# xiongzhenhai-zh/emqx

Measured on AMD Instinct MI355X. Metric: published topics matched/sec (and match evals/sec) at 10M subs; % of HBM BW, higher is better.
Workload: dtype u32; 1 GPU; B: 10M mixed exact/'+'/'#' subscriptions, 1xMI355X, batched topics of depth 4-8; n_filters=10000000, batch_topics_per_gpu=1000000, mode=routes, parallelism=replicated table, topic stream split x1, walk_order=batch order

## Files before the change

### emqx_amd/csrc/engine.cpp

```cpp
#include <hip/hip_runtime.h>

#include <algorithm>
#include <atomic>
#include <chrono>
#include <cstdlib>
#include <cstring>
#include <memory>
#include <mutex>
#include <string>
#include <thread>
#include <vector>

#include "../../include/emqx_match.h"
#include "kernels.h"
#include "streams.h"
#include "tables.h"

using namespace emqx;

namespace {

#define HIP_TRY(expr)                    \
  do {                                   \
    hipError_t _e = (expr);              \
// ... 99 lines not shown
  uint32_t deep_slab_cap = 1u << 20;
  uint64_t* h_rb = nullptr;
  bool deep_ready = false;
  bool ordered = false;
  hipEvent_t evo = nullptr;
  uint64_t ord_cap_n = 0, ord_cap_bytes = 0, ord_temp_bytes = 0;
  uint64_t* ord_keys = nullptr;
  uint64_t* ord_keys_out = nullptr;
  uint32_t* ord_idx = nullptr;
  uint32_t* ord_perm = nullptr;
  uint32_t* ord_lens = nullptr;
  uint32_t* ord_corig = nullptr;
  uint64_t* ord_noffs = nullptr;
  uint64_t* ord_partials = nullptr;
  uint8_t* ord_bytes = nullptr;
  uint8_t* ord_temp = nullptr;

  ~Workspace() {
    (void)hipSetDevice(device);
    dfree(counts); dfree(deferred); dfree(deep_rank); dfree(slab); dfree(tile_fill);
    dfree(tile_defer); dfree(spill); dfree(diag); dfree(ctrl); dfree(tile_sum); dfree(tile_stats);
    dfree(group_sum); dfree(group_stats);
    dfree(deep_wids); dfree(deep_stack); dfree(deep_slab);
    dfree(ord_keys); dfree(ord_keys_out); dfree(ord_idx); dfree(ord_perm); dfree(ord_lens); dfree(ord_corig);
    dfree(ord_noffs); dfree(ord_partials); dfree(ord_bytes); dfree(ord_temp);
    if (h_rb) (void)hipHostFree(h_rb);
    if (ev0) (void)hipEventDestroy(ev0);
    if (ev1) (void)hipEventDestroy(ev1);
    if (evk) (void)hipEventDestroy(evk);
    if (evo) (void)hipEventDestroy(evo);
    if (done) (void)hipEventDestroy(done);
    if (stream) (void)hipStreamDestroy(stream);
  }
};

uint64_t round_pow2(uint64_t x) {
  uint64_t p = 1;
  while (p < x) p <<= 1;
  return p;
}

}

struct emqx_engine {
  int device = 0;
  std::mutex writer;
  FilterStore store;
  uint64_t epoch = 0;
  double last_build_ms = 0;
  std::mutex snap_mu;
  std::shared_ptr<Snapshot> snap;
  std::mutex ws_mu;
  std::vector<std::unique_ptr<Workspace>> all_ws;
  std::vector<Workspace*> free_ws;
  std::atomic<uint64_t> last_evals{0}, last_deferred{0}, last_max_stack{0};
  std::atomic<double> last_match_ms{0};
  std::atomic<double> last_kernel_ms{0};
  std::atomic<int> forced_variant{-1};
  std::atomic<bool> diag_on{false};
  std::atomic<uint32_t> diag_stop{0};
  uint4* timeline = nullptr;
  uint64_t timeline_cap = 0;
  std::atomic<uint32_t> slab_hint{256};
  LiveState ls;
  std::vector<uint32_t> dirty;
  bool incremental = true;
  int64_t delta_max = -1;
  uint64_t last_commit_kind = 0;
  uint64_t last_relocations = 0, last_in_place = 0, last_patches = 0, last_new_slots = 0;
  double last_host_ms = 0;
  uint64_t last_extents = 0, last_vocab_slots = 0;
  double last_upload_ms = 0;
  std::mutex hb_mu;
  std::vector<emqx_host_batch*> hb_free;
  int commit_threads = std::max(1u, std::min(8u, std::thread::hardware_concurrency()));
  std::atomic<int> order{-1};
  std::atomic<int> order_level_bits{0};
  std::atomic<int> order_sort_bits{64};
  std::atomic<int> order_deal{1};
  std::atomic<uint64_t> last_ordered{0};
  std::atomic<uint64_t> order_bpt{48};
  std::atomic<double> last_order_ms{0};
  std::atomic<bool> small_batch{true};
};

namespace {

constexpr int EMQX_NEED_FULL = 1;

void publish(emqx_engine* e, std::shared_ptr<Snapshot> s) {
  std::lock_guard<std::mutex> g(e->snap_mu);
  e->snap = std::move(s);
}

int full_commit(emqx_engine* e) {
  auto vs = std::make_unique<VocabState>();
  std::vector<uint64_t> loc;
  std::vector<uint32_t> slot_ids;
  BuildOpts o;
  o.vocab = vs.get();
  o.fid_loc = &loc;
  o.slot_ids = &slot_ids;
  o.threads = e->commit_threads;
  HostTables ht;
  std::string err;
  if (!build_tables(e->store, o, ht, &err)) {
    set_last_error(err.c_str());
    return EMQX_ENOMEM;
  }
  const uint64_t n_slots = ht.edges.size();
  const uint64_t spare = std::min<uint64_t>(std::max<uint64_t>(1u << 20, n_slots / 2), MAX_SLOTS - n_slots);
  auto dt = std::make_shared<DeviceTables>();
  dt->device = e->device;
  dt->cap_slots = n_slots + spare;
  dt->n_vocab = ht.vocab.size();
  dt->cap_arena = ht.arena.size() + std::max<uint64_t>(1u << 20, ht.arena.size() / 4) + 16;
  HIP_TRY(dalloc(dt->edges, dt->cap_slots));
  HIP_TRY(dalloc(dt->fids, 2 * dt->cap_slots));
  HIP_TRY(dalloc(dt->vocab, dt->n_vocab));
  HIP_TRY(dalloc(dt->arena, dt->cap_arena));
  HIP_TRY(hipMemcpy(dt->edges, ht.edges.data(), n_slots * sizeof(EdgeSlot), hipMemcpyHostToDevice));
  HIP_TRY(hipMemcpy(dt->fids, ht.fids.data(), ht.fids.size() * sizeof(uint32_t), hipMemcpyHostToDevice));
  HIP_TRY(hipMemcpy(dt->vocab, ht.vocab.data(), ht.vocab.size() * sizeof(VocabSlot), hipMemcpyHostToDevice));
  HIP_TRY(hipMemcpy(dt->arena, ht.arena.data(), ht.arena.size(), hipMemcpyHostToDevice));
  HIP_TRY(hipStreamSynchronize(nullptr));

  auto s = std::make_shared<Snapshot>();
  s->dt = dt;
  s->tv.edges = dt->edges;
  s->tv.fids = dt->fids;
  s->tv.vocab = dt->vocab;
  s->tv.arena = dt->arena;
  s->tv.vocab_mask = ht.vocab_mask;
  s->tv.root_base = ht.root_base;
  s->tv.root_meta = ht.root_meta;
  s->tv.root_hash_fid = ht.root_hash_fid;
  s->tv.plus_mask = ht.plus_mask;
  s->n_nodes = ht.n_nodes;
  s->n_slots = n_slots;
  s->n_words = ht.n_words;
  s->max_depth = ht.max_depth;
  s->bytes = dt->bytes();
  uint32_t max_id = 0;
  for (uint32_t x : e->store.ext) max_id = std::max(max_id, x);
  s->narrow = slab_narrow_ok(max_id);

  LiveState& d = e->ls;
  d.device = e->device;
  d.dt = dt;
  d.vocab = std::move(vs);
  if (!d.lt) d.lt = std::make_unique<LiveTrie>();
  d.lt->adopt(ht, loc, slot_ids, spare, d.vocab.get());
  d.valid = true;
  d.inserted = 0;
  d.base_live = e->store.n_live;
  e->dirty.clear();
  publish(e, std::move(s));
  e->last_commit_kind = 0;
  return EMQX_OK;
}

int live_commit(emqx_engine* e) {
  LiveState& d = e->ls;
  LiveTrie& lt = *d.lt;
  const FilterStore& fs = e->store;
  std::vector<uint32_t> ids(e->dirty);
// ... 125 lines not shown
    HIP_TRY(dalloc(w->ctrl, CTRL_WORDS));
    HIP_TRY(dalloc(w->diag, DIAG_WORDS));
    HIP_TRY(hipMemset(w->diag, 0, DIAG_WORDS * sizeof(uint64_t)));
  }
  if (!w->deep_ready) {
    HIP_TRY(dalloc(w->deep_wids, uint64_t(DEEP_WAVES) * DEEP_MAX_LEVELS));
    HIP_TRY(dalloc(w->deep_stack, uint64_t(DEEP_WAVES) * w->deep_stack_cap));
    HIP_TRY(dalloc(w->deep_slab, w->deep_slab_cap));
    w->deep_ready = true;
  }
  if (n > w->cap_n) {
    const uint64_t cap = round_pow2(std::max<uint64_t>(n, 1024));
    HIP_TRY(dalloc(w->counts, cap));
    HIP_TRY(dalloc(w->deferred, cap));
    HIP_TRY(dalloc(w->deep_rank, cap));
    w->cap_n = cap;
  }
  const uint64_t ntiles = (n + TILE_TOPICS - 1) / TILE_TOPICS;
  if (ntiles > w->cap_tiles || w->cap_tiles == 0) {
    const uint64_t cap = round_pow2(std::max<uint64_t>(ntiles, 64));
    HIP_TRY(dalloc(w->tile_fill, cap));
    HIP_TRY(dalloc(w->tile_defer, cap));
    HIP_TRY(dalloc(w->tile_sum, cap));
    HIP_TRY(dalloc(w->tile_stats, cap));
    HIP_TRY(dalloc(w->group_sum, cap / GROUP_TILES + 1));
    HIP_TRY(dalloc(w->group_stats, cap / GROUP_TILES + 1));
    HIP_TRY(dalloc(w->spill, cap * w->spill_cap));
    w->cap_tiles = cap;
  }
  const uint64_t need_slab = std::max<uint64_t>(ntiles, 1) * w->slab_per_tile * entry_bytes;
  if (need_slab > w->cap_slab) {
    const uint64_t cap = need_slab;
    HIP_TRY(dalloc(w->slab, cap));
    w->cap_slab = cap;
  }
  return EMQX_OK;
}

constexpr uint64_t ORDER_MIN_N = 65536;

bool use_order(const emqx_engine* e, const Snapshot& snap, uint64_t n) {
  if (n > 0xFFFFFFFFull) return false;
  const int o = e->order.load();
  if (o >= 0) return o > 0 && n > 0;
  return snap.max_depth > 12 && n >= ORDER_MIN_N;
}

int ensure_order(emqx_engine* e, Workspace* w, uint64_t n, uint32_t sort_bits) {
  if (n > w->ord_cap_n) {
    const uint64_t cap = round_pow2(std::max<uint64_t>(n, 1024));
    HIP_TRY(dalloc(w->ord_keys, cap));
    HIP_TRY(dalloc(w->ord_keys_out, cap));
    HIP_TRY(dalloc(w->ord_idx, cap));
    HIP_TRY(dalloc(w->ord_perm, cap));
    HIP_TRY(dalloc(w->ord_lens, cap));
    HIP_TRY(dalloc(w->ord_corig, cap));
    HIP_TRY(dalloc(w->ord_noffs, cap + 1));
    HIP_TRY(dalloc(w->ord_partials, scan_partials(cap)));
    w->ord_cap_n = cap;
  }
  const uint64_t tb = order_sort_temp_bytes(n, sort_bits);
  if (!w->ord_temp || tb > w->ord_temp_bytes) {
    HIP_TRY(dalloc(w->ord_temp, tb));
    w->ord_temp_bytes = tb;
  }
  const uint64_t want = e->order_bpt.load() * n + 4096;
  if (!w->ord_bytes || w->ord_cap_bytes < want) {
    const uint64_t cap = std::max<uint64_t>(w->ord_cap_bytes, want);
    HIP_TRY(dalloc(w->ord_bytes, cap + 16));
    w->ord_cap_bytes = cap;
  }
  return EMQX_OK;
}

FastVariant pick_variant(const emqx_engine* e, const Snapshot& snap) {
  static const int env_forced = [] {
    const char* v = getenv("EMQX_FAST_VARIANT");
    return v ? atoi(v) : -1;
  }();
  const int fv = e->forced_variant.load();
  const int forced = fv >= 0 ? fv : env_forced;
  if (forced >= 0 && forced < FAST_NVARIANTS) return static_cast<FastVariant>(forced);
  return snap.max_depth > 12 ? FAST_K1_S512W : FAST_K1_S384B1;
}

MatchArgs match_args(emqx_engine* e, const Snapshot& snap, Workspace* w, uint32_t mode, const uint8_t* d_tbytes,
                     const uint64_t* d_toffs, uint64_t n, uint64_t* d_out_off, uint32_t* d_out_ids, uint64_t cap,
                     uint64_t* summary) {
  MatchArgs a{};
  a.tv = snap.tv;
  a.tbytes = d_tbytes;
  a.toffs = d_toffs;
  a.n = n;
  a.mode = mode;
  a.slab_cap = w->slab_per_tile;
  a.counts = w->counts;
  a.slab = w->slab;
  a.narrow = snap.narrow ? 1u : 0u;
  a.tile_fill = w->tile_fill;
  a.tile_defer = w->tile_defer;
  a.spill = w->spill;
  a.diag = e->diag_on.load() ? w->diag : nullptr;
  a.diag_stop = a.diag ? e->diag_stop.load() : 0u;
  a.timeline = a.diag && e->timeline && (n + TILE_TOPICS - 1) / TILE_TOPICS <= e->timeline_cap ? e->timeline : nullptr;
  a.spill_cap = w->spill_cap;
  a.ctrl = w->ctrl;
  a.deferred = w->deferred;
  a.deep_wids = w->deep_wids;
  a.deep_stack = w->deep_stack;
  a.deep_stack_cap = w->deep_stack_cap;
  a.deep_waves = DEEP_WAVES;
  a.deep_slab = w->deep_slab;
  a.deep_slab_cap = w->deep_slab_cap;
  a.tile_sum = w->tile_sum;
  a.tile_stats = w->tile_stats;
  a.group_sum = w->group_sum;
  a.group_stats = w->group_stats;
  a.ngroups = static_cast<uint32_t>((n + TILE_TOPICS * GROUP_TILES - 1) / (TILE_TOPICS * GROUP_TILES));
  a.deep_rank = w->deep_rank;
  a.out_off = d_out_off;
  a.out_ids = d_out_ids;
  a.out_cap = d_out_ids ? cap : 0;
  a.summary = summary;
  return a;
}

uint64_t slab_entry_bytes(const Snapshot& snap) {
  return snap.narrow ? sizeof(SlabNarrow::T) : sizeof(SlabWide::T);
}

int enqueue_match(emqx_engine* e, const Snapshot& snap, Workspace* w, uint32_t mode, const uint8_t* d_tbytes,
                  const uint64_t* d_toffs, uint64_t n, uint64_t* d_out_off, uint32_t* d_out_ids, uint64_t cap,
                  uint64_t* summary, hipStream_t s) {
  int rc = ensure_ws(w, n, slab_entry_bytes(snap));
  if (rc != EMQX_OK) return rc;
  MatchArgs a = match_args(e, snap, w, mode, d_tbytes, d_toffs, n, d_out_off, d_out_ids, cap, summary);
  const bool ordered = use_order(e, snap, n);
  const uint32_t sort_bits = static_cast<uint32_t>(std::min(64, std::max(1, e->order_sort_bits.load())));
  if (ordered) {
    rc = ensure_order(e, w, n, sort_bits);
    if (rc != EMQX_OK) return rc;
  }

  HIP_TRY(hipStreamWaitEvent(s, w->done, 0));
  w->last_stream = s;
  HIP_TRY(hipMemsetAsync(w->ctrl, 0, CTRL_WORDS * sizeof(uint32_t), s));
  w->ordered = ordered;
  if (ordered) {
    HIP_TRY(hipEventRecord(w->evo, s));
    OrderArgs o{};
    o.tbytes = d_tbytes;
    o.toffs = d_toffs;
    o.n = n;
    const int lb = e->order_level_bits.load();
    o.level_bits = static_cast<uint32_t>(lb > 0 ? std::min(lb, 32) : (snap.max_depth > 12 ? 4 : 8));
    o.sort_bits = sort_bits;
    o.keys = w->ord_keys;
    o.keys_out = w->ord_keys_out;
    o.idx = w->ord_idx;
    o.perm = w->ord_perm;
    o.lens = w->ord_lens;
    o.noffs = w->ord_noffs;
    o.partials = w->ord_partials;
    o.obytes = w->ord_bytes;
    o.cap_bytes = w->ord_cap_bytes;
    o.temp = w->ord_temp;
    o.temp_bytes = w->ord_temp_bytes;
    o.ctrl = w->ctrl;
    HIP_TRY(launch_order(o, s));
    a.tbytes = w->ord_bytes;
    a.toffs = w->ord_noffs;
    a.perm = w->ord_perm;
    a.deal = e->order_deal.load() ? 1u : 0u;
    a.corig = w->ord_corig;
    a.partials = w->ord_partials;
  }
  HIP_TRY(hipEventRecord(w->ev0, s));
  HIP_TRY(launch_match_fast(a, pick_variant(e, snap), s));
  HIP_TRY(hipEventRecord(w->evk, s));
  HIP_TRY(launch_match_deep(a, s));
  HIP_TRY(launch_assemble(a, s));
  HIP_TRY(hipEventRecord(w->ev1, s));
  HIP_TRY(hipEventRecord(w->done, s));
  return EMQX_OK;
}

int run_match(emqx_engine* e, const Snapshot& snap, Workspace* w, uint32_t mode, const uint8_t* d_tbytes,
              const uint64_t* d_toffs, uint64_t n, uint64_t* d_out_off, uint32_t* d_out_ids, uint64_t cap,
              uint64_t* n_out, hipStream_t s) {
  uint64_t* sum_dev = nullptr;
  HIP_TRY(hipHostGetDevicePointer(reinterpret_cast<void**>(&sum_dev), w->h_rb, 0));
  for (int attempt = 0; attempt < 8; ++attempt) {
    int rc = enqueue_match(e, snap, w, mode, d_tbytes, d_toffs, n, d_out_off, d_out_ids, cap, sum_dev, s);
    if (rc != EMQX_OK) return rc;
    HIP_TRY(hipStreamSynchronize(s));
    const uint64_t* sm = w->h_rb;
    const uint64_t flags = sm[SUM_FLAGS];
    const uint32_t err = static_cast<uint32_t>(sm[SUM_ERROR]);
    if (flags & SUM_F_ERROR) {
      set_last_error("topic longer than 65535 bytes on the deep path");
      return EMQX_EINVAL;
    }
    if (flags & SUM_F_RETRY) {
      if (sm[SUM_NEED_SLAB] > w->slab_per_tile) {
        const uint64_t need = sm[SUM_NEED_SLAB];
// ... 607 lines not shown
  }
  auto s = current(e);
  if (s) {
    out->n_nodes = s->n_nodes;
    out->n_slots = s->n_slots;
    out->n_words = s->n_words;
    out->table_bytes = s->bytes;
    out->max_depth = s->max_depth;
  }
  out->last_ordered = e->last_ordered.load();
  out->last_order_ms = e->last_order_ms.load();
  out->last_evals = e->last_evals.load();
  out->last_deferred = e->last_deferred.load();
  out->last_max_stack = e->last_max_stack.load();
  out->last_match_ms = e->last_match_ms.load();
  out->last_kernel_ms = e->last_kernel_ms.load();
  out->size = want;
  std::memcpy(dst, out, want);
  return EMQX_OK;
}

const char* emqx_strerror(int code) {
  switch (code) {
    case EMQX_OK: return "ok";
    case EMQX_EINVAL: return "invalid argument";
    case EMQX_ENOMEM: return "out of memory";
    case EMQX_EDEVICE: return g_last_error.empty() ? "device error" : g_last_error.c_str();
    case EMQX_EOVERFLOW: return "output capacity too small";
    case EMQX_ENOTFOUND: return "not found";
    case EMQX_ETOODEEP: return "topic frontier too deep";
    case EMQX_EBUSY: return "busy: every batch buffer is in use";
    default: return "unknown error";
  }
}

int emqx_set_tuning(emqx_engine* e, const char* key, int64_t value) {
  if (!e || !key) return EMQX_EINVAL;
  if (std::strcmp(key, "fast_variant") == 0) {
    if (value < -1 || value >= FAST_NVARIANTS) return EMQX_EINVAL;
    e->forced_variant.store(static_cast<int>(value));
    return EMQX_OK;
  }
  if (std::strcmp(key, "diag") == 0) {
    e->diag_on.store(value != 0);
    return EMQX_OK;
  }
  if (std::strcmp(key, "diag_stop") == 0) {
    e->diag_stop.store(static_cast<uint32_t>(value));
    return EMQX_OK;
  }
  if (std::strcmp(key, "timeline") == 0) {
    if (value < 0) return EMQX_EINVAL;
    HIP_TRY(hipSetDevice(e->device));
    HIP_TRY(hipDeviceSynchronize());
    dfree(e->timeline);
    e->timeline_cap = 0;
    if (value) {
      HIP_TRY(dalloc(e->timeline, static_cast<uint64_t>(value)));
      HIP_TRY(hipMemset(e->timeline, 0, static_cast<uint64_t>(value) * sizeof(uint4)));
      e->timeline_cap = static_cast<uint64_t>(value);
    }
    return EMQX_OK;
  }
  if (std::strcmp(key, "small_batch") == 0) {
    e->small_batch.store(value != 0);
    return EMQX_OK;
  }
  if (std::strcmp(key, "incremental") == 0) {
    std::lock_guard<std::mutex> g(e->writer);
    e->incremental = value != 0;
    return EMQX_OK;
  }
  if (std::strcmp(key, "commit_threads") == 0) {
    if (value < 1 || value > 256) return EMQX_EINVAL;
    std::lock_guard<std::mutex> g(e->writer);
    e->commit_threads = static_cast<int>(value);
    return EMQX_OK;
  }
  if (std::strcmp(key, "order") == 0) {
    if (value < -1 || value > 1) return EMQX_EINVAL;
    e->order.store(static_cast<int>(value));
    return EMQX_OK;
  }
  if (std::strcmp(key, "order_level_bits") == 0) {
    if (value < 0 || value > 32) return EMQX_EINVAL;
    e->order_level_bits.store(static_cast<int>(value));
    return EMQX_OK;
  }
  if (std::strcmp(key, "order_sort_bits") == 0) {
    if (value < 1 || value > 64) return EMQX_EINVAL;
    e->order_sort_bits.store(static_cast<int>(value));
    return EMQX_OK;
  }
  if (std::strcmp(key, "order_deal") == 0) {
    e->order_deal.store(value != 0);
    return EMQX_OK;
  }
  if (std::strcmp(key, "delta_max") == 0) {
    std::lock_guard<std::mutex> g(e->writer);
    e->delta_max = value;
    return EMQX_OK;
  }
  return EMQX_ENOTFOUND;
}

uint64_t emqx_permute_scratch_bytes(uint64_t n) { return permute_scratch_bytes(n); }

uint64_t emqx_owner_sort_scratch_bytes(uint64_t n, uint32_t world) { return owner_sort_scratch_bytes(n, world); }

int emqx_owner_sort_device(const uint32_t* d_owner, uint64_t n, uint32_t world, uint32_t* d_perm, void* d_scratch,
                           void* stream) {
  if (world == 0 || (n && (!d_owner || !d_perm || !d_scratch)) || n > 0xFFFFFFFFull) return EMQX_EINVAL;
  HIP_TRY(launch_owner_sort(d_owner, n, world, d_perm, d_scratch, static_cast<hipStream_t>(stream)));
  return EMQX_OK;
}

int emqx_batch_permute_device(const uint8_t* d_bytes, const uint64_t* d_offsets, uint64_t n, const uint32_t* d_perm,
                              uint8_t* d_out_bytes, uint64_t* d_out_offsets, void* d_scratch, void* stream) {
  if (!d_out_offsets || !d_scratch || (n && (!d_bytes || !d_offsets || !d_perm || !d_out_bytes))) return EMQX_EINVAL;
  HIP_TRY(launch_batch_permute(d_bytes, d_offsets, n, d_perm, d_out_bytes, d_out_offsets, d_scratch,
                               static_cast<hipStream_t>(stream)));
  return EMQX_OK;
}

int emqx_csr_unpermute_device(const uint32_t* d_counts, const uint32_t* d_ids, uint64_t n, const uint32_t* d_perm,
                              uint64_t* d_out_offsets, uint32_t* d_out_ids, void* d_scratch, void* stream) {
  if (!d_out_offsets || !d_scratch || (n && (!d_counts || !d_perm))) return EMQX_EINVAL;
  HIP_TRY(launch_csr_unpermute(d_counts, d_ids, n, d_perm, d_out_offsets, d_out_ids, d_scratch,
                               static_cast<hipStream_t>(stream)));
  return EMQX_OK;
}

int emqx_shard_owner_device(const uint8_t* d_bytes, const uint64_t* d_offsets, uint64_t n, uint32_t world,
                            uint32_t levels, uint32_t* d_owner, void* stream) {
  if ((n && (!d_bytes || !d_offsets || !d_owner)) || world == 0 || levels == 0) return EMQX_EINVAL;
  HIP_TRY(launch_shard_owner(d_bytes, d_offsets, n, world, levels, d_owner, static_cast<hipStream_t>(stream)));
  return EMQX_OK;
}

int emqx_shard_route_device(const uint8_t* d_bytes, const uint64_t* d_offsets, uint64_t n, uint32_t world,
                            const emqx_shard_split* d_splits, uint32_t n_splits, uint32_t* d_req2, void* stream) {
  if ((n && (!d_bytes || !d_offsets || !d_req2)) || world == 0 || (n_splits && !d_splits)) return EMQX_EINVAL;
  HIP_TRY(launch_shard_route(d_bytes, d_offsets, n, world, reinterpret_cast<const ShardSplitE*>(d_splits), n_splits,
                             d_req2, static_cast<hipStream_t>(stream)));
  return EMQX_OK;
}

int emqx_commit_stats(emqx_engine* e, uint64_t* out, uint32_t n) {
  if (!e || (n && !out)) return EMQX_EINVAL;
  std::lock_guard<std::mutex> g(e->writer);
  const LiveTrie* lt = e->ls.lt.get();
  uint64_t host_us = static_cast<uint64_t>(e->last_host_ms * 1e3);
  const uint64_t v[12] = {e->last_commit_kind, e->last_relocations, e->last_in_place, e->last_patches,
                          e->last_new_slots, lt ? lt->used : 0, lt ? lt->cap : 0, lt ? lt->garbage : 0, host_us,
                          e->last_extents, e->last_vocab_slots, static_cast<uint64_t>(e->last_upload_ms * 1e3)};
  for (uint32_t i = 0; i < n && i < 12; ++i) out[i] = v[i];
  return EMQX_OK;
}

int emqx_diag_read(emqx_engine* e, uint64_t* out, uint32_t n, int reset) {
  if (!e || !out) return EMQX_EINVAL;
  HIP_TRY(hipSetDevice(e->device));
  std::vector<uint64_t> acc(DIAG_WORDS, 0), tmp(DIAG_WORDS);
  std::lock_guard<std::mutex> g(e->ws_mu);
  for (auto& w : e->all_ws) {
    if (!w->diag) continue;
// ... 22 lines not shown
```

### emqx_amd/csrc/kernels.h

```cpp
#pragma once

#include <hip/hip_runtime.h>
#include <stdint.h>

#include "layout.h"

namespace emqx {

enum Ctrl : uint32_t {
  CTRL_DEFERRED = 0,
  CTRL_NEED_SLAB = 1,
  CTRL_ERROR = 2,
  CTRL_DEEP_FILL = 3,
  CTRL_DEEP_EVALS = 4,
  CTRL_WORDS = 8
};
constexpr uint32_t GROUP_TILES = 256;
constexpr uint32_t CTRL_ERR_TOO_LONG = 1u;
constexpr uint32_t CTRL_ERR_TOO_DEEP = 2u;
constexpr uint32_t CTRL_ERR_DEEP_SLAB = 4u;
constexpr uint32_t CTRL_ERR_ORDER_CAP = 8u;

constexpr int TILE_TOPICS = 64;

enum Diag : uint32_t {
  DIAG_STEPS = 0,
  DIAG_ITEMS = 1,
  DIAG_LIT_PROBES = 2,
  DIAG_LIT_HITS = 3,
  DIAG_LIT_EXTRA = 4,
  DIAG_PLUS_PROBES = 5,
  DIAG_PLUS_HITS = 6,
  DIAG_EMITS = 7,
  DIAG_SPILLS = 8,
  DIAG_TICKS_A = 9,
  DIAG_TICKS_B = 10,
  DIAG_WAVES = 11,
  DIAG_LEVEL0 = 12,
  DIAG_SMALL = 20,
  DIAG_WIDE = 21,
  DIAG_NCOUNT = 22,
  DIAG_WORDS = 32
};
constexpr uint32_t DEEP_MAX_LEVELS = 65536;

enum Summary : uint32_t {
  SUM_FLAGS = 0,
  SUM_TOTAL = 1,
  SUM_EVALS = 2,
  SUM_MAXSTACK = 3,
  SUM_DEFERRED = 4,
  SUM_NEED_SLAB = 5,
  SUM_DEEP_FILL = 6,
  SUM_ERROR = 7,
  SUM_WORDS = 8
};
constexpr uint64_t SUM_F_RETRY = 1;
constexpr uint64_t SUM_F_OVERFLOW = 2;
constexpr uint64_t SUM_F_ERROR = 4;

struct MatchArgs {
  TableView tv;
  const uint8_t* tbytes;
  const uint64_t* toffs;
  uint64_t n;
  uint32_t mode;
  uint32_t slab_cap;
  uint32_t* counts;
  void* slab;
  uint32_t narrow;
  uint32_t* tile_fill;
  uint64_t* tile_defer;
  uint32_t* ctrl;
  uint32_t* deferred;
  uint64_t* diag;
  uint4* timeline;
  uint32_t diag_stop;
  uint2* spill;
  uint32_t spill_cap;
  uint32_t* deep_wids;
  uint4* deep_stack;
  uint32_t deep_stack_cap;
  uint32_t deep_waves;
  uint64_t* deep_slab;
  uint32_t deep_slab_cap;
  uint64_t* tile_sum;
  uint2* tile_stats;
  uint64_t* group_sum;
  uint2* group_stats;
  uint32_t ngroups;
  uint32_t* deep_rank;
  uint64_t* out_off;
  uint32_t* out_ids;
  uint64_t out_cap;
  uint64_t* summary;
  const uint32_t* perm;
  uint32_t deal;
  uint32_t* corig;
  uint64_t* partials;
};

constexpr uint32_t SMALL_WAVES = 16;
constexpr uint64_t SMALL_MAX_N = uint64_t(SMALL_WAVES) * TILE_TOPICS;
constexpr uint32_t SMALL_FO_MAX_ENTRIES = 16384;

struct SmallFanout {
  const uint4* recs;
  uint32_t n_recs;
  const uint32_t* plain;
  const uint4* groups;
  const uint32_t* members;
  uint32_t strategy;
  uint32_t seed;
  const uint32_t* h_keys;
  uint32_t* d_keys;
  uint4* erec;
  uint32_t* etop;
  const unsigned long long* ps_count;
  uint64_t* h_off;
  uint32_t* h_subs;
  uint32_t* h_fil;
  uint64_t cap;
  uint64_t* h_sum;
};

struct SmallArgs {
  MatchArgs m;
  const uint8_t* h_tbytes;
  const uint64_t* h_toffs;
  uint64_t nbytes;
  uint32_t tt;
  uint32_t slab_tiles;
  uint32_t has_fanout;
  uint64_t* h_out_off;
  uint32_t* h_out_ids;
  uint64_t h_cap;
  uint64_t* clk;
  SmallFanout f;
};
enum : uint32_t {
  SMALL_CLK_COPY = 0, SMALL_CLK_WALK, SMALL_CLK_DEEP, SMALL_CLK_SCAN, SMALL_CLK_SCATTER, SMALL_CLK_OUT,
  SMALL_CLK_FO_PASS1, SMALL_CLK_FO_PASS2, SMALL_CLK_LAUNCHES, SMALL_CLK_WORDS = 10
};
hipError_t launch_small_batch(const SmallArgs& a, hipStream_t s);
}
struct emqx_engine;
namespace emqx {
constexpr int SMALL_NOT_TAKEN = 1;
int engine_small_batch(emqx_engine* e, uint32_t mode, const uint8_t* h_tbytes, const uint64_t* h_toffs, uint64_t n,
                       uint64_t nbytes, uint8_t* d_tbytes, uint64_t* d_toffs, uint64_t* d_out_off, uint32_t* d_out_ids,
                       uint64_t cap, uint64_t* h_summary, const SmallFanout& f, hipStream_t s);

constexpr uint32_t DEEP_WAVES = 512;
constexpr uint32_t DEEP_CHUNK = 256;
constexpr uint64_t DEEP_PAD = ~0ull;

enum FastVariant {
  FAST_K1_S1K = 0,
  FAST_K2_S1K = 1,
  FAST_K2_S2K = 2,
  FAST_K2_S768 = 3,
  FAST_K4_S2K = 4,
  FAST_K1_S256 = 5,
  FAST_K2_S512 = 6,
  FAST_K1_S384 = 7,
  FAST_K2_S512W = 8,
  FAST_K1_S768W = 9,
  FAST_K1_S512W = 10,
  FAST_K1_S384R = 11,
  FAST_K1_S384P = 12,
  FAST_K1_S384N = 13,
  FAST_K1_S384W7 = 14,
  FAST_K1_S384B2 = 15,
  FAST_K1_S384B1 = 16,
  FAST_K1_S512WB1 = 17,
  FAST_NVARIANTS = 18
};
// ... 49 lines not shown
```

### emqx_amd/csrc/layout.h

```cpp
#pragma once

#include <stdint.h>

#if defined(__HIPCC__)
#define EMQX_HD __host__ __device__ __forceinline__
#else
#define EMQX_HD inline
#endif

namespace emqx {

constexpr uint32_t WID_NONE = 0xFFFFFFFFu;
constexpr uint32_t WID_PLUS = 0xFFFFFFFEu;
constexpr uint32_t WID_HASH = 0xFFFFFFFDu;
constexpr uint32_t FID_NONE = 0xFFFFFFFFu;

constexpr uint32_t META_CAPLOG2_MASK = 0x1Fu;
constexpr uint32_t META_HAS_PLUS = 1u << 5;
constexpr uint32_t META_HAS_EDGES = 1u << 6;
constexpr uint32_t META_HAS_HASH = 1u << 7;
constexpr uint32_t META_HAS_TERM = 1u << 8;
constexpr uint32_t META_TERM_WILD = 1u << 9;
constexpr uint32_t META_PH = 1u << 10;
constexpr uint32_t META_LITF_EXACT = 1u << 11;
constexpr uint32_t META_LITF_NONE = 1u << 12;
constexpr uint32_t META_BUCKET_OVF = 1u << 13;
constexpr uint32_t META_XFID = 1u << 14;
constexpr uint32_t META_XFID_TERM = 1u << 15;
constexpr uint32_t META_F8_SHIFT = 24;
constexpr uint32_t META_SEED_SHIFT = 16;
constexpr uint32_t PH_MAX_CAPLOG = 15;

struct alignas(16) EdgeSlot {
  uint32_t wid;
  uint32_t child_base;
  uint32_t meta;
  uint32_t litf;
};
static_assert(sizeof(EdgeSlot) == 16, "EdgeSlot must be 16 bytes");
constexpr uint64_t MAX_SLOTS = (1ull << 31) - 1;

constexpr uint32_t SLAB_NARROW_ID_BITS = 26;
constexpr uint32_t SLAB_NARROW_IDS = (1u << SLAB_NARROW_ID_BITS) - 1u;
EMQX_HD bool slab_narrow_ok(uint32_t max_id) { return max_id < SLAB_NARROW_IDS; }
struct SlabWide {
  typedef uint64_t T;
  static constexpr T PAD = ~0ull;
  static EMQX_HD T make(uint32_t owner, uint32_t id) { return (static_cast<uint64_t>(owner) << 32) | id; }
  static EMQX_HD uint32_t owner(T e) { return static_cast<uint32_t>(e >> 32) & 63u; }
  static EMQX_HD uint32_t id(T e) { return static_cast<uint32_t>(e); }
};
struct SlabNarrow {
  typedef uint32_t T;
  static constexpr T PAD = ~0u;
  static EMQX_HD T make(uint32_t owner, uint32_t id) { return (owner << SLAB_NARROW_ID_BITS) | id; }
  static EMQX_HD uint32_t owner(T e) { return e >> SLAB_NARROW_ID_BITS; }
  static EMQX_HD uint32_t id(T e) { return e & ((1u << SLAB_NARROW_ID_BITS) - 1u); }
};

struct alignas(16) SlotPatch {
  uint32_t slot;
  uint32_t fid_h, fid_t;
  uint32_t pad;
  EdgeSlot s;
};
static_assert(sizeof(SlotPatch) == 32, "SlotPatch must be 32 bytes");

struct alignas(16) VocabSlot {
  uint32_t hash;
  uint32_t len;
  uint32_t wid;
  uint32_t off;
  uint32_t inl[4];
};
static_assert(sizeof(VocabSlot) == 32, "VocabSlot must be 32 bytes");

struct TableView {
  const EdgeSlot* edges;
  const uint32_t* fids;
  const VocabSlot* vocab;
  const uint8_t* arena;
  uint32_t vocab_mask;
  uint32_t root_base;
  uint32_t root_meta;
  uint32_t root_hash_fid;
  uint32_t plus_mask;
};

constexpr uint32_t PLUS_LINE = 4;
constexpr uint32_t PLUS_COPY_MAX_CAPLOG = 14;
EMQX_HD bool plus_copies(uint32_t plus_mask, bool has_plus, uint32_t caplog) {
  return plus_mask != 0 && has_plus && caplog > 2 && caplog <= PLUS_COPY_MAX_CAPLOG;
}
EMQX_HD bool plus_position(uint32_t i, bool copies) { return copies ? (i & (PLUS_LINE - 1u)) == 0 : i == 0; }
EMQX_HD uint32_t plus_copy(uint32_t i1, bool copies) { return copies ? (i1 & ~(PLUS_LINE - 1u)) : 0u; }

EMQX_HD uint32_t mix32(uint32_t x) {
  x ^= x >> 16;
  x *= 0x85ebca6bu;
  x ^= x >> 13;
  x *= 0xc2b2ae35u;
  x ^= x >> 16;
  return x;
}

EMQX_HD uint32_t whash_init(uint32_t len) { return len * 0x9E3779B1u + 0x7F4A7C15u; }
EMQX_HD uint32_t whash_step(uint32_t h, uint32_t d) {
  h = (h ^ d) * 0x85EBCA77u;
  return (h << 13) | (h >> 19);
}
EMQX_HD uint32_t word_hash16(uint32_t len, uint32_t w0, uint32_t w1, uint32_t w2, uint32_t w3) {
  return mix32(whash_step(whash_step(whash_step(whash_step(whash_init(len), w0), w1), w2), w3));
}
EMQX_HD uint32_t word_hash_bytes(const uint8_t* p, uint32_t n) {
  uint32_t h = whash_init(n);
  const uint32_t nd = n > 16 ? (n + 3) / 4 : 4;
  for (uint32_t i = 0; i < nd; ++i) {
    uint32_t d = 0;
    for (uint32_t b = 0; b < 4; ++b)
      if (4 * i + b < n) d |= static_cast<uint32_t>(p[4 * i + b]) << (8 * b);
    h = whash_step(h, d);
  }
  return mix32(h);
}

EMQX_HD uint32_t vocab_slot0(uint32_t hash) { return hash; }

EMQX_HD uint32_t node_hash(uint32_t wid, uint32_t seed) { return mix32(wid ^ (seed * 0x9E3779B1u + 0x7F4A7C15u)); }

EMQX_HD uint32_t ph_slot(uint32_t h, uint32_t mask, bool copies) {
  const uint32_t s = h & mask;
  return (!copies || (s & (PLUS_LINE - 1u))) ? s : s + 1u + (h >> 31);
}
EMQX_HD uint32_t lit_slot(uint32_t wid, uint32_t seed, uint32_t mask, bool copies) {
  return ph_slot(node_hash(wid, seed), mask, copies);
}


EMQX_HD uint32_t bucket1(uint32_t wid, uint32_t seed, uint32_t nbmask) { return node_hash(wid, seed) & nbmask; }
EMQX_HD uint32_t bucket2(uint32_t wid, uint32_t seed, uint32_t nbmask) {
  const uint32_t a = bucket1(wid, seed, nbmask), b = mix32(wid ^ (0xDAA66D2Bu + seed * 0x7F4A7C15u)) & nbmask;
// ... 201 lines not shown
```

### emqx_amd/csrc/match_kernels.hip

```cpp
#include <hip/hip_runtime.h>

#include <algorithm>

#include "fanout.h"
#include "kernels.h"

namespace emqx {

namespace {

constexpr uint32_t MODE_ROUTES = 0, MODE_TRIE = 1;

__device__ __forceinline__ uint32_t lane_id() {
  return __builtin_amdgcn_mbcnt_hi(~0u, __builtin_amdgcn_mbcnt_lo(~0u, 0u));
}

__device__ __forceinline__ void wave_sync() {
  __builtin_amdgcn_fence(__ATOMIC_SEQ_CST, "wavefront");
  __builtin_amdgcn_wave_barrier();
}

__device__ __forceinline__ uint64_t lanemask_lt(uint32_t lane) { return (1ull << lane) - 1ull; }

template <int BITS>
// ... 1198 lines not shown
#pragma unroll
  for (int k = 0; k < SCAN_ITEMS; ++k) {
    const uint64_t i = base + k;
    v[k] = i < n ? counts[i] : 0u;
    s += v[k];
  }
  uint64_t tot;
  uint64_t run = partials[blockIdx.x] + block_excl_scan(s, &tot);
#pragma unroll
  for (int k = 0; k < SCAN_ITEMS; ++k) {
    const uint64_t i = base + k;
    if (i < n) offsets[i] = run;
    run += v[k];
  }
}

__global__ __launch_bounds__(SCAN_THREADS) void scan_single_kernel(const uint32_t* counts, uint64_t n,
                                                                   uint64_t* offsets) {
  const uint64_t base = static_cast<uint64_t>(threadIdx.x) * SCAN_ITEMS;
  uint32_t v[SCAN_ITEMS];
  uint64_t s = 0;
#pragma unroll
  for (int k = 0; k < SCAN_ITEMS; ++k) {
    const uint64_t i = base + k;
    v[k] = i < n ? counts[i] : 0u;
    s += v[k];
  }
  uint64_t tot;
  uint64_t run = block_excl_scan(s, &tot);
#pragma unroll
  for (int k = 0; k < SCAN_ITEMS; ++k) {
    const uint64_t i = base + k;
    if (i < n) offsets[i] = run;
    run += v[k];
  }
  if (threadIdx.x == 0) offsets[n] = tot;
}

__device__ __forceinline__ uint64_t wave_sum64(uint64_t v) {
#pragma unroll
  for (uint32_t d = 32; d >= 1; d >>= 1)
    v += (static_cast<uint64_t>(__shfl_xor(static_cast<uint32_t>(v >> 32), d, 64)) << 32) |
         __shfl_xor(static_cast<uint32_t>(v), d, 64);
  return v;
}

__global__ __launch_bounds__(GROUP_TILES) void group_reduce_kernel(MatchArgs a, uint64_t ntiles) {
  __shared__ uint64_t ws[GROUP_TILES / 64], we[GROUP_TILES / 64];
  __shared__ uint32_t wm[GROUP_TILES / 64];
  const uint32_t lane = threadIdx.x & 63, w = threadIdx.x >> 6;
  const uint64_t i = static_cast<uint64_t>(blockIdx.x) * GROUP_TILES + threadIdx.x;
  uint64_t v = 0, ev = 0;
  uint32_t mx = 0;
  if (i < ntiles) {
    v = a.tile_sum[i];
    const uint2 st = a.tile_stats[i];
    ev = st.x;
    mx = st.y;
  }
  v = wave_sum64(v);
  ev = wave_sum64(ev);
  for (uint32_t d = 32; d >= 1; d >>= 1) mx = max(mx, static_cast<uint32_t>(__shfl_xor(mx, d, 64)));
  if (lane == 0) {
    ws[w] = v;
    we[w] = ev;
    wm[w] = mx;
  }
  __syncthreads();
  if (threadIdx.x == 0) {
    uint64_t sv = 0, se = 0;
    uint32_t sm = 0;
    for (uint32_t k = 0; k < GROUP_TILES / 64; ++k) {
      sv += ws[k];
      se += we[k];
      sm = max(sm, wm[k]);
    }
    a.group_sum[blockIdx.x] = sv;
    a.group_stats[blockIdx.x] = make_uint2(static_cast<uint32_t>(min<uint64_t>(se, 0xFFFFFFFFull)), sm);
  }
}

template <class E>
__device__ __forceinline__ void scatter_tile(const MatchArgs& a, uint64_t tile, uint64_t off);

template <class E>
__global__ __launch_bounds__(256) void scatter_fast_kernel(MatchArgs a) {
  const uint32_t lane = lane_id();
  const uint32_t wv = threadIdx.x >> 6;
  const uint64_t tile = static_cast<uint64_t>(blockIdx.x) * 4 + wv;
  const uint64_t t0 = tile * TILE_TOPICS;
  if (t0 >= a.n) return;
  const uint64_t t = t0 + lane;
  uint64_t off = 0;
  if (a.perm) {
    if (a.ctrl[CTRL_ERROR] & CTRL_ERR_ORDER_CAP) return;
    off = t < a.n ? a.out_off[a.perm[t]] : 0;
  } else {
    const uint64_t g = tile / GROUP_TILES, g0 = g * GROUP_TILES;
    uint64_t before = 0;
    for (uint64_t k = lane; k < g; k += 64) before += a.group_sum[k];
    for (uint64_t j = g0 + lane; j < tile; j += 64) before += a.tile_sum[j];
    before = wave_sum64(before);
    const uint64_t c = t < a.n ? a.counts[t] : 0;
    off = before + wave_incl_scan64(c, lane) - c;
    if (t < a.n) a.out_off[t] = off;
  }
  scatter_tile<E>(a, tile, off);
}

template <class E>
__device__ __forceinline__ void scatter_tile(const MatchArgs& a, uint64_t tile, uint64_t off) {
  typedef typename E::T T;
  const uint32_t lane = lane_id();
  uint64_t next = off;
  const uint32_t fill = min(a.tile_fill[tile], a.slab_cap);
  const uint64_t dmask = a.tile_defer[tile];
  const T* slab = static_cast<const T*>(a.slab) + tile * a.slab_cap;
  const uint64_t lt = lanemask_lt(lane);
  constexpr uint32_t U = 32 / sizeof(T);
  for (uint32_t i0 = 0; i0 < fill; i0 += 64 * U) {
    T e[U];
#pragma unroll
    for (uint32_t u = 0; u < U; ++u) {
      const uint32_t i = i0 + 64 * u + lane;
      e[u] = i < fill ? slab[i] : E::PAD;
    }
#pragma unroll
    for (uint32_t u = 0; u < U; ++u) {
      if (i0 + 64 * u >= fill) break;
      const uint32_t tl = E::owner(e[u]);
      const bool keep = e[u] != E::PAD && !((dmask >> tl) & 1ull);
      const uint64_t km = __ballot(keep);
      uint64_t peers = km, mine = km;
#pragma unroll
      for (uint32_t bit = 0; bit < 6; ++bit) {
        const uint64_t m = __ballot(keep && ((tl >> bit) & 1u));
        peers &= ((tl >> bit) & 1u) ? m : ~m;
        mine &= ((lane >> bit) & 1u) ? m : ~m;
      }
      const uint32_t rk = static_cast<uint32_t>(__popcll(peers & lt));
      const uint32_t lo = __shfl(static_cast<uint32_t>(next), static_cast<int>(tl), 64);
      const uint32_t hi = __shfl(static_cast<uint32_t>(next >> 32), static_cast<int>(tl), 64);
      if (keep) {
        const uint64_t p = ((static_cast<uint64_t>(hi) << 32) | lo) + rk;
        if (p < a.out_cap) a.out_ids[p] = E::id(e[u]);
      }
      next += static_cast<uint64_t>(__popcll(mine));
    }
  }
}

__global__ __launch_bounds__(64) void summary_kernel(MatchArgs a) {
  const uint32_t lane = lane_id();
  uint64_t tot = 0, ev = 0;
  uint32_t mx = 0;
  for (uint32_t k = lane; k < a.ngroups; k += 64) {
    tot += a.group_sum[k];
    const uint2 st = a.group_stats[k];
    ev += st.x;
    mx = max(mx, st.y);
  }
  tot = wave_sum64(tot);
  ev = wave_sum64(ev);
  for (uint32_t d = 32; d >= 1; d >>= 1) mx = max(mx, static_cast<uint32_t>(__shfl_xor(mx, d, 64)));
  if (lane == 0) {
    const uint32_t* c = a.ctrl;
    const uint32_t need = c[CTRL_NEED_SLAB], err = c[CTRL_ERROR];
    uint64_t flags = 0;
    if (need > a.slab_cap || (err & (CTRL_ERR_DEEP_SLAB | CTRL_ERR_TOO_DEEP | CTRL_ERR_ORDER_CAP))) flags |= SUM_F_RETRY;
    if (tot > a.out_cap) flags |= SUM_F_OVERFLOW;
    if (err & CTRL_ERR_TOO_LONG) flags |= SUM_F_ERROR;
    a.out_off[a.n] = tot;
    uint64_t* sm = a.summary;
    sm[SUM_TOTAL] = tot;
    sm[SUM_EVALS] = ev + c[CTRL_DEEP_EVALS];
    sm[SUM_MAXSTACK] = mx;
    sm[SUM_DEFERRED] = c[CTRL_DEFERRED];
    sm[SUM_NEED_SLAB] = need;
    sm[SUM_DEEP_FILL] = c[CTRL_DEEP_FILL];
    sm[SUM_ERROR] = err;
    sm[SUM_FLAGS] = flags;
    __threadfence_system();
  }
}

__global__ __launch_bounds__(256) void scatter_deep_kernel(MatchArgs a) {
  const uint32_t fill = min(a.ctrl[CTRL_DEEP_FILL], a.deep_slab_cap);
  for (uint64_t i = static_cast<uint64_t>(blockIdx.x) * blockDim.x + threadIdx.x; i < fill;
       i += static_cast<uint64_t>(gridDim.x) * blockDim.x) {
    const uint64_t e = a.deep_slab[i];
    if (e == DEEP_PAD) continue;
    const uint32_t j = static_cast<uint32_t>(e >> 32) & 0x7FFFFFFFu;
    const uint32_t t = a.deferred[j];
    const uint64_t p = a.out_off[a.perm ? a.perm[t] : t] + atomicAdd(&a.deep_rank[j], 1u);
    if (p < a.out_cap) a.out_ids[p] = resolve_entry(a.tv, e);
  }
}

__global__ __launch_bounds__(256) void csr_to_host_kernel(const uint64_t* __restrict__ d_off, uint64_t n,
                                                          const uint32_t* __restrict__ d_ids, uint64_t cap,
                                                          uint64_t* h_off, uint32_t* h_ids) {
  const uint64_t tid = static_cast<uint64_t>(blockIdx.x) * blockDim.x + threadIdx.x;
  const uint64_t nt = static_cast<uint64_t>(gridDim.x) * blockDim.x;
  const uint64_t total = min(d_off[n], cap);
  const uint64_t no2 = (n + 1) / 2;
  for (uint64_t i = tid; i < no2; i += nt)
    reinterpret_cast<uint4*>(h_off)[i] = reinterpret_cast<const uint4*>(d_off)[i];
  if (tid == 0 && ((n + 1) & 1)) h_off[n] = d_off[n];
  const uint64_t nv = total / 4;
  for (uint64_t i = tid; i < nv; i += nt)
    reinterpret_cast<uint4*>(h_ids)[i] = reinterpret_cast<const uint4*>(d_ids)[i];
  if (tid < total - 4 * nv) h_ids[4 * nv + tid] = d_ids[4 * nv + tid];
}

__global__ __launch_bounds__(256) void shard_owner_kernel(const uint8_t* __restrict__ tbytes,
                                                          const uint64_t* __restrict__ toffs, uint64_t n,
                                                          uint32_t world, uint32_t levels,
                                                          uint32_t* __restrict__ owner) {
  for (uint64_t i = static_cast<uint64_t>(blockIdx.x) * blockDim.x + threadIdx.x; i < n;
       i += static_cast<uint64_t>(gridDim.x) * blockDim.x) {
    const uint64_t a = toffs[i], b = toffs[i + 1];
    owner[i] = shard_owner(tbytes + a, b - a, world, levels, true);
  }
}

__global__ void slot_patch_kernel(EdgeSlot* edges, uint32_t* fids, const SlotPatch* patches, uint32_t n,
                                  int phase) {
  for (uint32_t i = blockIdx.x * blockDim.x + threadIdx.x; i < n; i += gridDim.x * blockDim.x) {
    const SlotPatch& p = patches[i];
    if (phase == 0) {
      *reinterpret_cast<uint2*>(fids + 2ull * p.slot) = make_uint2(p.fid_h, p.fid_t);
// ... 287 lines not shown
      hipLaunchKernelGGL((match_fast_kernel<W, S, WC, K, false, RL, 0, NH, SlabWide>), grid, block, 0, s, a);
  }
}

hipError_t launch_match_fast(const MatchArgs& a, FastVariant v, hipStream_t s) {
  const uint64_t ntiles = (a.n + TILE_TOPICS - 1) / TILE_TOPICS;
  if (ntiles == 0) return hipSuccess;
  switch (v) {
    case FAST_K1_S1K: launch_fast_t<4, 1024, 1024, 1>(a, ntiles, s); break;
    case FAST_K2_S1K: launch_fast_t<4, 1024, 1024, 2>(a, ntiles, s); break;
    case FAST_K2_S2K: launch_fast_t<2, 2048, 1024, 2>(a, ntiles, s); break;
    case FAST_K2_S768: launch_fast_t<4, 768, 768, 2>(a, ntiles, s); break;
    case FAST_K4_S2K: launch_fast_t<2, 2048, 1024, 4>(a, ntiles, s); break;
    case FAST_K1_S256: launch_fast_t<4, 256, 512, 1>(a, ntiles, s); break;
    case FAST_K2_S512: launch_fast_t<4, 512, 640, 2>(a, ntiles, s); break;
    case FAST_K1_S384: launch_fast_t<4, 384, 640, 1>(a, ntiles, s); break;
    case FAST_K2_S512W: launch_fast_t<4, 512, 512, 2>(a, ntiles, s); break;
    case FAST_K1_S768W: launch_fast_t<4, 768, 1024, 1>(a, ntiles, s); break;
    case FAST_K1_S512W: launch_fast_t<4, 512, 1024, 1>(a, ntiles, s); break;
    case FAST_K1_S384R: launch_fast_t<4, 384, 640, 1, true>(a, ntiles, s); break;
    case FAST_K1_S384N: launch_fast_t<4, 384, 640, 1, false, false>(a, ntiles, s); break;
    case FAST_K1_S384W7: launch_fast_t<4, 384, 448, 1>(a, ntiles, s); break;
    case FAST_K1_S384B2: launch_fast_t<2, 384, 640, 1>(a, ntiles, s); break;
    case FAST_K1_S384B1: launch_fast_t<1, 384, 640, 1>(a, ntiles, s); break;
    case FAST_K1_S512WB1: launch_fast_t<1, 512, 1024, 1>(a, ntiles, s); break;
    case FAST_K1_S384P: {
      if (a.diag) {
        launch_fast_t<4, 384, 640, 1>(a, ntiles, s);
        break;
      }
      const dim3 grid(static_cast<uint32_t>((ntiles + 3) / 4));
      hipLaunchKernelGGL((match_fast_kernel<4, 384, 640, 1, false, false, 1>), grid, dim3(256), 0, s, a);
      if (a.narrow)
        hipLaunchKernelGGL((match_fast_kernel<4, 384, 640, 1, false, false, 2, true, SlabNarrow>), grid, dim3(256), 0, s, a);
      else
        hipLaunchKernelGGL((match_fast_kernel<4, 384, 640, 1, false, false, 2>), grid, dim3(256), 0, s, a);
      break;
    }
    default: return hipErrorInvalidValue;
  }
  return hipGetLastError();
}

hipError_t launch_small_batch(const SmallArgs& a, hipStream_t s) {
  const uint64_t tiles = a.tt ? (a.m.n + a.tt - 1) / a.tt : 0;
  if (a.m.n == 0 || a.m.n > SMALL_MAX_N || a.tt == 0 || a.tt > TILE_TOPICS || tiles > SMALL_WAVES ||
      tiles > a.slab_tiles || a.m.narrow)
    return hipErrorInvalidValue;
  hipLaunchKernelGGL(small_batch_kernel, dim3(1), dim3(SMALL_WAVES * 64), 0, s, a);
  return hipGetLastError();
}

hipError_t launch_match_deep(const MatchArgs& a, hipStream_t s) {
  const uint32_t blocks = (a.deep_waves * 64 + 255) / 256;
  hipLaunchKernelGGL(match_deep_kernel, dim3(blocks), dim3(256), 0, s, a);
  return hipGetLastError();
}

uint64_t scan_partials(uint64_t n) { return (n + SCAN_TILE - 1) / SCAN_TILE + 1; }

hipError_t launch_scan(const uint32_t* counts, uint64_t n, uint64_t* offsets, uint64_t* partials,
                       hipStream_t s) {
  const uint64_t nb = (n + SCAN_TILE - 1) / SCAN_TILE;
  if (nb <= 1) {
    hipLaunchKernelGGL(scan_single_kernel, dim3(1), dim3(SCAN_THREADS), 0, s, counts, n, offsets);
    return hipGetLastError();
  }
  hipLaunchKernelGGL(scan_reduce_kernel, dim3(static_cast<uint32_t>(nb)), dim3(SCAN_THREADS), 0, s, counts, n, partials);
  hipLaunchKernelGGL(scan_partials_kernel, dim3(1), dim3(SCAN_THREADS), 0, s, partials, nb, offsets, n);
  hipLaunchKernelGGL(scan_final_kernel, dim3(static_cast<uint32_t>(nb)), dim3(SCAN_THREADS), 0, s, counts, n, partials, offsets);
  return hipGetLastError();
}

hipError_t launch_assemble(const MatchArgs& a, hipStream_t s) {
  const uint64_t ntiles = (a.n + TILE_TOPICS - 1) / TILE_TOPICS;
  if (ntiles) {
    hipLaunchKernelGGL(group_reduce_kernel, dim3(a.ngroups), dim3(GROUP_TILES), 0, s, a, ntiles);
    if (a.perm) {
      hipError_t err = launch_order_counts(a.counts, a.perm, a.n, a.corig, s);
      if (err == hipSuccess) err = launch_scan(a.corig, a.n, a.out_off, a.partials, s);
      if (err != hipSuccess) return err;
    }
    const dim3 grid(static_cast<uint32_t>((ntiles + 3) / 4));
    if (a.narrow)
      hipLaunchKernelGGL(scatter_fast_kernel<SlabNarrow>, grid, dim3(256), 0, s, a);
    else
      hipLaunchKernelGGL(scatter_fast_kernel<SlabWide>, grid, dim3(256), 0, s, a);
  }
  hipLaunchKernelGGL(scatter_deep_kernel, dim3(64), dim3(256), 0, s, a);
  hipLaunchKernelGGL(summary_kernel, dim3(1), dim3(64), 0, s, a);
  return hipGetLastError();
}

hipError_t launch_csr_to_host(const uint64_t* d_off, uint64_t n, const uint32_t* d_ids, uint64_t cap,
                               uint64_t* h_off, uint32_t* h_ids, hipStream_t s) {
  const uint64_t work = std::max<uint64_t>((n + 1) / 2, cap / 4);
  const uint32_t blocks = static_cast<uint32_t>(std::min<uint64_t>((work + 255) / 256 + 1, 2048));
  hipLaunchKernelGGL(csr_to_host_kernel, dim3(blocks), dim3(256), 0, s, d_off, n, d_ids, cap, h_off, h_ids);
  return hipGetLastError();
}

hipError_t launch_shard_owner(const uint8_t* tbytes, const uint64_t* toffs, uint64_t n, uint32_t world,
                              uint32_t levels, uint32_t* owner, hipStream_t s) {
  if (!n) return hipSuccess;
  const uint32_t blocks = static_cast<uint32_t>(std::min<uint64_t>((n + 255) / 256, 4096));
  hipLaunchKernelGGL(shard_owner_kernel, dim3(blocks), dim3(256), 0, s, tbytes, toffs, n, world, levels, owner);
  return hipGetLastError();
}

hipError_t launch_slot_patches(EdgeSlot* edges, uint32_t* fids, const SlotPatch* patches, uint32_t n,
                               hipStream_t s) {
  if (!n) return hipSuccess;
  const dim3 grid(std::min<uint32_t>((n + 255) / 256, 1024));
  hipLaunchKernelGGL(slot_patch_kernel, grid, dim3(256), 0, s, edges, fids, patches, n, 0);
  hipLaunchKernelGGL(slot_patch_kernel, grid, dim3(256), 0, s, edges, fids, patches, n, 1);
  return hipGetLastError();
}

}
```

Baseline: 1.899 billion topics/s.

## Stage tile scatter output in LDS window and write coalesced 16-byte vectors

```diff
diff --git a/emqx_amd/csrc/engine.cpp b/emqx_amd/csrc/engine.cpp
--- a/emqx_amd/csrc/engine.cpp
+++ b/emqx_amd/csrc/engine.cpp
@@ -205,6 +205,7 @@
   std::atomic<uint64_t> order_bpt{48};
   std::atomic<double> last_order_ms{0};
   std::atomic<bool> small_batch{true};
+  std::atomic<int> scatter_stage{-1};
 };
 
 namespace {
@@ -496,6 +497,17 @@
   const int forced = fv >= 0 ? fv : env_forced;
   if (forced >= 0 && forced < FAST_NVARIANTS) return static_cast<FastVariant>(forced);
   return snap.max_depth > 12 ? FAST_K1_S512W : FAST_K1_S384B1;
+}
+
+bool use_scatter_stage(const emqx_engine* e, const Snapshot& snap, uint32_t slab_per_tile) {
+  static const int env_forced = [] {
+    const char* v = getenv("EMQX_SCATTER_STAGE");
+    return v ? atoi(v) : -1;
+  }();
+  const int tv = e->scatter_stage.load();
+  const int forced = tv >= 0 ? tv : env_forced;
+  if (forced >= 0) return forced != 0;
+  return snap.max_depth <= 12 && slab_per_tile > 256;
 }
 
 MatchArgs match_args(emqx_engine* e, const Snapshot& snap, Workspace* w, uint32_t mode, const uint8_t* d_tbytes,
@@ -535,6 +547,7 @@
   a.out_off = d_out_off;
   a.out_ids = d_out_ids;
   a.out_cap = d_out_ids ? cap : 0;
+  a.scatter_stage = use_scatter_stage(e, snap, a.slab_cap) ? 1u : 0u;
   a.summary = summary;
   return a;
 }
@@ -1308,6 +1321,11 @@
     e->order.store(static_cast<int>(value));
     return EMQX_OK;
   }
+  if (std::strcmp(key, "scatter_stage") == 0) {
+    if (value < -1 || value > 1) return EMQX_EINVAL;
+    e->scatter_stage.store(static_cast<int>(value));
+    return EMQX_OK;
+  }
   if (std::strcmp(key, "order_level_bits") == 0) {
     if (value < 0 || value > 32) return EMQX_EINVAL;
     e->order_level_bits.store(static_cast<int>(value));
diff --git a/emqx_amd/csrc/kernels.h b/emqx_amd/csrc/kernels.h
--- a/emqx_amd/csrc/kernels.h
+++ b/emqx_amd/csrc/kernels.h
@@ -22,6 +22,9 @@
 constexpr uint32_t CTRL_ERR_ORDER_CAP = 8u;
 
 constexpr int TILE_TOPICS = 64;
+
+constexpr uint32_t SCATTER_STAGE_W = 1024;
+constexpr uint32_t SCATTER_STAGE_P = 8;
 
 enum Diag : uint32_t {
   DIAG_STEPS = 0,
@@ -93,6 +96,7 @@
   uint64_t* out_off;
   uint32_t* out_ids;
   uint64_t out_cap;
+  uint32_t scatter_stage;
   uint64_t* summary;
   const uint32_t* perm;
   uint32_t deal;
diff --git a/emqx_amd/csrc/layout.h b/emqx_amd/csrc/layout.h
--- a/emqx_amd/csrc/layout.h
+++ b/emqx_amd/csrc/layout.h
@@ -57,6 +57,18 @@
   static EMQX_HD uint32_t owner(T e) { return e >> SLAB_NARROW_ID_BITS; }
   static EMQX_HD uint32_t id(T e) { return e & ((1u << SLAB_NARROW_ID_BITS) - 1u); }
 };
+
+struct SpanSplit {
+  uint32_t head, vecs, tail;
+};
+EMQX_HD SpanSplit span_split(uint64_t addr, uint32_t len) {
+  const uint32_t to_boundary = static_cast<uint32_t>((16u - (addr & 15u)) & 15u) >> 2;
+  SpanSplit s;
+  s.head = to_boundary < len ? to_boundary : len;
+  s.vecs = (len - s.head) >> 2;
+  s.tail = len - s.head - 4u * s.vecs;
+  return s;
+}
 
 struct alignas(16) SlotPatch {
   uint32_t slot;
diff --git a/emqx_amd/csrc/match_kernels.hip b/emqx_amd/csrc/match_kernels.hip
--- a/emqx_amd/csrc/match_kernels.hip
+++ b/emqx_amd/csrc/match_kernels.hip
@@ -1304,6 +1304,22 @@
 
 template <class E>
 __device__ __forceinline__ void scatter_tile(const MatchArgs& a, uint64_t tile, uint64_t off);
+template <class E>
+__device__ __forceinline__ void scatter_tile_staged(const MatchArgs& a, uint64_t tile, uint64_t base, uint32_t rel,
+                                                    uint32_t tsum, uint32_t* win);
+
+__device__ __forceinline__ uint64_t tile_offsets(const MatchArgs& a, uint64_t tile, uint32_t lane) {
+  const uint64_t t = tile * TILE_TOPICS + lane;
+  const uint64_t g = tile / GROUP_TILES, g0 = g * GROUP_TILES;
+  uint64_t before = 0;
+  for (uint64_t k = lane; k < g; k += 64) before += a.group_sum[k];
+  for (uint64_t j = g0 + lane; j < tile; j += 64) before += a.tile_sum[j];
+  before = wave_sum64(before);
+  const uint64_t c = t < a.n ? a.counts[t] : 0;
+  const uint64_t off = before + wave_incl_scan64(c, lane) - c;
+  if (t < a.n) a.out_off[t] = off;
+  return off;
+}
 
 template <class E>
 __global__ __launch_bounds__(256) void scatter_fast_kernel(MatchArgs a) {
@@ -1318,16 +1334,39 @@
     if (a.ctrl[CTRL_ERROR] & CTRL_ERR_ORDER_CAP) return;
     off = t < a.n ? a.out_off[a.perm[t]] : 0;
   } else {
-    const uint64_t g = tile / GROUP_TILES, g0 = g * GROUP_TILES;
-    uint64_t before = 0;
-    for (uint64_t k = lane; k < g; k += 64) before += a.group_sum[k];
-    for (uint64_t j = g0 + lane; j < tile; j += 64) before += a.tile_sum[j];
-    before = wave_sum64(before);
-    const uint64_t c = t < a.n ? a.counts[t] : 0;
-    off = before + wave_incl_scan64(c, lane) - c;
-    if (t < a.n) a.out_off[t] = off;
+    off = tile_offsets(a, tile, lane);
   }
   scatter_tile<E>(a, tile, off);
+}
+
+template <class E>
+__global__ __launch_bounds__(64) void scatter_staged_kernel(MatchArgs a) {
+  __shared__ __attribute__((aligned(16))) uint32_t win[SCATTER_STAGE_W + 4];
+  const uint32_t lane = lane_id();
+  const uint64_t tile = blockIdx.x;
+  const uint64_t off = tile_offsets(a, tile, lane);
+  const uint64_t base = (static_cast<uint64_t>(__shfl(static_cast<uint32_t>(off >> 32), 0, 64)) << 32) |
+                        __shfl(static_cast<uint32_t>(off), 0, 64);
+  const uint64_t tsum = a.tile_sum[tile];
+  const bool staged = a.tile_defer[tile] == 0 && a.tile_fill[tile] <= a.slab_cap &&
+                      tsum <= static_cast<uint64_t>(SCATTER_STAGE_P) * SCATTER_STAGE_W && base + tsum <= a.out_cap;
+  if (staged)
+    scatter_tile_staged<E>(a, tile, base, static_cast<uint32_t>(off - base), static_cast<uint32_t>(tsum), win);
+  else
+    scatter_tile<E>(a, tile, off);
+}
+
+__device__ __forceinline__ uint32_t round_ranks(bool keep, uint32_t tl, uint32_t lane, uint64_t lt, uint32_t* cnt) {
+  const uint64_t km = __ballot(keep);
+  uint64_t peers = km, mine = km;
+#pragma unroll
+  for (uint32_t bit = 0; bit < 6; ++bit) {
+    const uint64_t m = __ballot(keep && ((tl >> bit) & 1u));
+    peers &= ((tl >> bit) & 1u) ? m : ~m;
+    mine &= ((lane >> bit) & 1u) ? m : ~m;
+  }
+  *cnt = static_cast<uint32_t>(__popcll(mine));
+  return static_cast<uint32_t>(__popcll(peers & lt));
 }
 
 template <class E>
@@ -1352,23 +1391,64 @@
       if (i0 + 64 * u >= fill) break;
       const uint32_t tl = E::owner(e[u]);
       const bool keep = e[u] != E::PAD && !((dmask >> tl) & 1ull);
-      const uint64_t km = __ballot(keep);
-      uint64_t peers = km, mine = km;
-#pragma unroll
-      for (uint32_t bit = 0; bit < 6; ++bit) {
-        const uint64_t m = __ballot(keep && ((tl >> bit) & 1u));
-        peers &= ((tl >> bit) & 1u) ? m : ~m;
-        mine &= ((lane >> bit) & 1u) ? m : ~m;
-      }
-      const uint32_t rk = static_cast<uint32_t>(__popcll(peers & lt));
+      uint32_t cnt;
+      const uint32_t rk = round_ranks(keep, tl, lane, lt, &cnt);
       const uint32_t lo = __shfl(static_cast<uint32_t>(next), static_cast<int>(tl), 64);
       const uint32_t hi = __shfl(static_cast<uint32_t>(next >> 32), static_cast<int>(tl), 64);
       if (keep) {
         const uint64_t p = ((static_cast<uint64_t>(hi) << 32) | lo) + rk;
         if (p < a.out_cap) a.out_ids[p] = E::id(e[u]);
       }
-      next += static_cast<uint64_t>(__popcll(mine));
-    }
+      next += cnt;
+    }
+  }
+}
+
+template <class E>
+__device__ __forceinline__ void scatter_tile_staged(const MatchArgs& a, uint64_t tile, uint64_t base, uint32_t rel,
+                                                    uint32_t tsum, uint32_t* win) {
+  typedef typename E::T T;
+  constexpr uint32_t W = SCATTER_STAGE_W;
+  const uint32_t lane = lane_id();
+  const uint32_t fill = a.tile_fill[tile];
+  const T* slab = static_cast<const T*>(a.slab) + tile * a.slab_cap;
+  const uint64_t lt = lanemask_lt(lane);
+  constexpr uint32_t U = 32 / sizeof(T);
+  for (uint32_t w0 = 0; w0 < tsum; w0 += W) {
+    uint32_t* dst = a.out_ids + base + w0;
+    const uint32_t len = min(W, tsum - w0);
+    const uint64_t addr = reinterpret_cast<uint64_t>(dst);
+    const uint32_t mis = static_cast<uint32_t>(addr >> 2) & 3u;
+    uint32_t next = rel;
+    for (uint32_t i0 = 0; i0 < fill; i0 += 64 * U) {
+      T e[U];
+#pragma unroll
+      for (uint32_t u = 0; u < U; ++u) {
+        const uint32_t i = i0 + 64 * u + lane;
+        e[u] = i < fill ? slab[i] : E::PAD;
+      }
+#pragma unroll
+      for (uint32_t u = 0; u < U; ++u) {
+        if (i0 + 64 * u >= fill) break;
+        const uint32_t tl = E::owner(e[u]);
+        const bool keep = e[u] != E::PAD;
+        uint32_t cnt;
+        const uint32_t rk = round_ranks(keep, tl, lane, lt, &cnt);
+        const uint32_t d = __shfl(next, static_cast<int>(tl), 64) + rk - w0;
+        if (keep && d < len) win[mis + d] = E::id(e[u]);
+        next += cnt;
+      }
+    }
+    wave_sync();
+    const SpanSplit sp = span_split(addr, len);
+    if (lane < sp.head) dst[lane] = win[mis + lane];
+    for (uint32_t v = lane; v < sp.vecs; v += 64) {
+      const uint32_t i = sp.head + 4 * v;
+      *reinterpret_cast<uint4*>(dst + i) = *reinterpret_cast<const uint4*>(win + mis + i);
+    }
+    const uint32_t t0 = sp.head + 4 * sp.vecs;
+    if (lane < sp.tail) dst[t0 + lane] = win[mis + t0 + lane];
+    wave_sync();
   }
 }
 
@@ -1822,7 +1902,13 @@
       if (err != hipSuccess) return err;
     }
     const dim3 grid(static_cast<uint32_t>((ntiles + 3) / 4));
-    if (a.narrow)
+    if (a.scatter_stage && !a.perm) {
+      const dim3 tiles(static_cast<uint32_t>(ntiles));
+      if (a.narrow)
+        hipLaunchKernelGGL(scatter_staged_kernel<SlabNarrow>, tiles, dim3(64), 0, s, a);
+      else
+        hipLaunchKernelGGL(scatter_staged_kernel<SlabWide>, tiles, dim3(64), 0, s, a);
+    } else if (a.narrow)
       hipLaunchKernelGGL(scatter_fast_kernel<SlabNarrow>, grid, dim3(256), 0, s, a);
     else
       hipLaunchKernelGGL(scatter_fast_kernel<SlabWide>, grid, dim3(256), 0, s, a);
```

After: 1.938 billion topics/s, median of 6. 1.02x the previous value.
